# limeorange1102/multimodal-av-model

Hardware: AMD Instinct MI355X
Metric: utterances/sec (4 s clip, 25 fps 96x96 lip) at batch 64, full training step (higher is better)
Workload: dtype bf16; 1 GPU; BASELINE metric configuration (= configs[3]'s per-GPU batch): batch 64/GPU x 4 s (T_audio 64000, T_enc 199, 100 lip frames 96x96 x 2 speakers), wav2vec2-large + ResNet-18 + fusion BiLSTM + CTC + contrastive, fwd+bwd+Adam, random-init weights; variant=as_executed, global_batch=64, parallelism=dp1, audio_passes=2, wav2vec2_regularizers=hf-defaults (dropout 0.1, LayerDrop 0.1, SpecAugment 0.05)

## Files before the change

### include/av_hip.h

```cpp
#ifndef AV_HIP_H
#define AV_HIP_H
#ifdef __cplusplus
extern "C" {
#endif

#define AV_OK 0
#define AV_ERR_ARG 1
#define AV_ERR_LAUNCH 2

#define AV_F32 0
#define AV_BF16 1

#define AV_A_ROWMAJOR 0
#define AV_A_TRANS 1
#define AV_A_CONV2D 2
#define AV_A_CONV3D1 3
#define AV_B_NK 0
#define AV_B_KN 1
#define AV_ACT_NONE 0
#define AV_ACT_GELU 1
#define AV_ACT_MUL_GELU_GRAD 2
#define AV_ACT_GELU_GF 3
#define AV_ACT_MUL_AUX 4

// ... 79 lines not shown
                    int rows_per_batch, int ld, void* stream);
int av_softmax_bwd_rows(const void* p, int pdt, const float* dp, void* ds, int dsdt, long long rows, int cols,
                        float scale, int ld, void* stream);

int av_conv0_ln_gelu(const float* wav, const float* w, const float* bias, const float* gamma, const float* beta, void* out,
                     int out_dtype, int B, int T_in, int L_out, int C, int k, int stride, float eps, void* stream);

int av_lstm_fwd_step(const float* gx, const void* whh, void* hseq, float* cseq, void* gates, void* out_bt, int dtype,
                     int T, int B, int H, int s, void* stream);
int av_lstm_bwd_step(const void* dout, int dout_dtype, long long do_bs, long long do_ts, void* dgates, const void* whhT,
                     const void* gates, const float* cseq, float* dc, int dtype, int T, int B, int H, int s, void* stream);

#define AV_LSTM_COUNTER_INTS 1024
int av_lstm_fwd_layer(const float* gx, const void* whh, void* hseq, float* cseq, void* gates, void* out_bt, int* counters,
                      int T, int B, int H, void* stream);
int av_lstm_bwd_layer(const void* dout, int dout_dtype, long long do_bs, long long do_ts, void* dgates, const void* whhT,
                      const void* gates, const float* cseq, float* dc, int* counters, int T, int B, int H, void* stream);

int av_mask_downsample(const long long* mask, long long* out, int B, int Tin, int Tout, void* stream);
int av_fusion_gather_lerp_fwd(const float* feat, const long long* mask, int* ws_i32, float* out, long long* mask_out,
                              long long* lens, int B, int Ta, int Tv, int D, int groups, void* stream);
int av_fusion_gather_lerp_bwd(const float* dout, const int* ws_i32, float* dfeat, int B, int Ta, int Tv, int D, int groups,
                              void* stream);
int av_permute_bt(const void* in, int idt, void* out, int odt, int B, int T, int D, void* stream);
int av_gather_rows(const void* src, int sdt, const long long* idx, void* out, int odt, long long n, int D, void* stream);
int av_scatter_rows(const float* src, const long long* idx, float* out, long long n, int D, float alpha, int accumulate,
                    void* stream);
int av_class_order(const long long* mask, long long n, long long* order, void* stream);

int av_conv3d_front(const float* x, const void* w, void* y, float* stats, int B, int T, int H, int W, void* stream);
int av_conv3d_front_pool(const float* x, const void* w, void* ymax, void* ymin, float* stats, int B, int T, int H, int W, void* stream);
int av_bn_prelu_minmax(const void* ymax, const void* ymin, const float* scale, const float* shift, const float* slope, void* out, long long n,
                       void* stream);
int av_conv3x3_c64(const void* x, const void* w, void* y, float* stats, int n_img, int H, int W, const float* in_scale,
                   const float* in_shift, const float* in_slope, void* stream);
int av_bn_finalize(const float* partial, int nblk, long long count, const float* gamma, const float* beta,
                   float* running_mean, float* running_var, float momentum, float eps, int training, float* scale,
                   float* shift, int C, double* ws, int ws_zeroed, void* stream);
int av_bn_act(const void* x, const float* scale, const float* shift, const void* res, const float* rscale,
              const float* rshift, const float* slope, void* out, int dtype, long long n, int C, void* stream);
int av_bn_prelu_maxpool(const void* x, const float* scale, const float* shift, const float* slope, void* out, int dtype,
                        long long N, int H, int W, int C, void* stream);
int av_avgpool(const void* x, int dtype, float* out, long long N, int HW, int C, int pm_block, void* stream);

int av_l2norm_fwd(const float* x, float* y, float* nrm, long long rows, int cols, float eps, void* stream);
int av_l2norm_bwd(const float* y, const float* dy, const float* nrm, float* dx, long long rows, int cols, float eps,
                  void* stream);
int av_lse_rows(const float* s, float* lse, float* rowsum, long long rows, int cols, int ld, void* stream);
int av_contrastive_dsim(const float* s, const float* lse, void* out, int odt, long long rows, int cols, int ld, float coef,
                        void* stream);
int av_lse_rows_chunk(const float* s, float* lse, float* rowsum, long long rows, int cols, int ld, int accumulate, void* stream);
int av_contrastive_dsim_chunk(const float* s, const float* lse, void* out, int odt, long long rows, int cols, int ld, float coef,
                              int total_cols, void* stream);
int av_reduce_sum(const float* x, long long n, float* out, float scale, int accumulate, void* stream);
int av_loss_combine(const float* nll, const float* w, const float* c1, const float* c2, float half_lambda, int n, float* out3,
                    void* stream);
int av_ctc_greedy(const float* log_probs, const long long* lengths, int* out_ids, int* out_len, int B, int T, int V, int blank,
                  void* stream);
int av_ctc_beam_workspace_bytes(int B, int T, int V, int beam_width, long long* bytes);
int av_ctc_beam_frame_pass(const float* log_probs, long long stride_b, long long stride_t, const long long* lengths, void* workspace,
                           long long workspace_bytes, int B, int T, int V, int blank, int beam_width, void* stream);
int av_ctc_beam_search(const float* log_probs, long long stride_b, long long stride_t, const long long* lengths, int* out_ids,
                       int* out_len, float* out_score, void* workspace, long long workspace_bytes, int B, int T, int V, int blank,
                       int beam_width, int nbest, void* stream);
int av_ngram_score(const int* ids, const long long* lens, float* out, int B, int Lmax, const float* lm_unigrams, const void* lm_table,
                   long long lm_slots, int lm_order, int lm_vocab, int lm_bos, int lm_probe_bound, void* stream);
// ... 122 lines not shown
```

### multimodal-av-model_amd/_lib.py

```python
from __future__ import annotations

import ctypes as C
import os

from . import precision as _precision

_HERE = os.path.dirname(os.path.abspath(__file__))
LIB_PATH = os.environ.get("AVAMD_LIB") or os.path.join(_HERE, "libavhip.so")

AV_F32, AV_BF16 = 0, 1
A_ROWMAJOR, A_TRANS, A_CONV2D, A_CONV3D1 = 0, 1, 2, 3
B_NK, B_KN = 0, 1
ACT_NONE, ACT_GELU, ACT_MUL_GELU_GRAD, ACT_GELU_GF, ACT_MUL_AUX = 0, 1, 2, 3, 4
LSTM_COUNTER_INTS = 1024

vp, ll, i32, f32 = C.c_void_p, C.c_longlong, C.c_int, C.c_float


class GemmArgs(C.Structure):
    _fields_ = [
        ("A", vp), ("B", vp), ("C", vp), ("C2", vp), ("bias", vp), ("R", vp), ("aux", vp), ("stats", vp),
        ("M", i32), ("N", i32), ("K", i32), ("batch", i32),
        ("lda", ll), ("ldb", ll), ("ldc", ll), ("ldr", ll),
        ("sA", ll), ("sB", ll), ("sC", ll), ("sR", ll), ("sBias", ll),
# ... 52 lines not shown
    "av_log_softmax_bwd_ld": [vp, vp, vp, i32, ll, i32, i32, vp],
    "av_colsum": [vp, i32, vp, ll, i32, ll, i32, vp],
    "av_cast": [vp, i32, vp, i32, ll, vp],
    "av_cast_dropout": [vp, i32, vp, i32, ll, f32, C.c_ulonglong, C.c_uint, vp],
    "av_dropout_uniform": [vp, ll, C.c_ulonglong, C.c_uint, vp],
    "av_fusion_xattn_fwd": [vp, vp, vp, vp, vp, vp, vp, vp, i32, i32, i32, i32, f32, vp],
    "av_fusion_xattn_bwd": [vp, vp, vp, vp, vp, vp, vp, i32, i32, i32, i32, f32, vp],
    "av_zero_feature_cols": [vp, i32, vp, i32, i32, i32, vp],
    "av_overwrite_rows": [vp, i32, vp, vp, ll, i32, vp],
    "av_axpby": [f32, vp, i32, f32, vp, ll, vp],
    "av_mask_rows": [vp, i32, vp, ll, i32, vp],
    "av_mul_scalar_dev": [vp, vp, vp, ll, vp],
    "av_attention_fwd": [vp, vp, vp, vp, vp, i32, i32, i32, i32, i32, i32, ll, ll, ll, ll, ll, ll, ll, ll, vp, f32, f32, C.c_ulonglong, C.c_uint, vp],
    "av_attention_dropmask": [vp, i32, i32, i32, i32, f32, C.c_ulonglong, C.c_uint, vp],
    "av_attention_fwd_mask": [vp, vp, vp, vp, vp, i32, i32, i32, i32, i32, i32, ll, ll, ll, ll, ll, ll, ll, ll, vp, f32, f32, C.c_ulonglong, C.c_uint, vp, vp],
    "av_attention_bwd_mask": [vp, vp, vp, vp, vp, vp, vp, vp, vp, vp, i32, i32, i32, i32, i32, vp, vp, f32, f32, C.c_ulonglong, C.c_uint, vp, vp],
    "av_attention_bwd": [vp, vp, vp, vp, vp, vp, vp, vp, vp, vp, i32, i32, i32, i32, i32, vp, vp, f32, f32, C.c_ulonglong, C.c_uint, vp],
    "av_softmax_rows": [vp, vp, i32, ll, i32, f32, vp, i32, i32, vp],
    "av_conv0_ln_gelu": [vp, vp, vp, vp, vp, vp, i32, i32, i32, i32, i32, i32, i32, f32, vp],
    "av_lstm_fwd_step": [vp, vp, vp, vp, vp, vp, i32, i32, i32, i32, i32, vp],
    "av_lstm_bwd_step": [vp, i32, ll, ll, vp, vp, vp, vp, vp, i32, i32, i32, i32, i32, vp],
    "av_lstm_fwd_layer": [vp, vp, vp, vp, vp, vp, vp, i32, i32, i32, vp],
    "av_lstm_bwd_layer": [vp, i32, ll, ll, vp, vp, vp, vp, vp, vp, i32, i32, i32, vp],
    "av_mask_downsample": [vp, vp, i32, i32, i32, vp],
    "av_fusion_gather_lerp_fwd": [vp, vp, vp, vp, vp, vp, i32, i32, i32, i32, i32, vp],
    "av_fusion_gather_lerp_bwd": [vp, vp, vp, i32, i32, i32, i32, i32, vp],
    "av_permute_bt": [vp, i32, vp, i32, i32, i32, i32, vp],
    "av_gather_rows": [vp, i32, vp, vp, i32, ll, i32, vp],
    "av_scatter_rows": [vp, vp, vp, ll, i32, f32, i32, vp],
    "av_class_order": [vp, ll, vp, vp],
    "av_conv3d_front": [vp, vp, vp, vp, i32, i32, i32, i32, vp],
    "av_conv3d_front_pool": [vp, vp, vp, vp, vp, i32, i32, i32, i32, vp],
    "av_bn_prelu_minmax": [vp, vp, vp, vp, vp, vp, ll, vp],
    "av_conv3x3_c64": [vp, vp, vp, vp, i32, i32, i32, vp, vp, vp, vp],
    "av_bn_finalize": [vp, i32, ll, vp, vp, vp, vp, f32, f32, i32, vp, vp, i32, vp, i32, vp],
    "av_bn_act": [vp, vp, vp, vp, vp, vp, vp, vp, i32, ll, i32, vp],
    "av_bn_prelu_maxpool": [vp, vp, vp, vp, vp, i32, ll, i32, i32, i32, vp],
    "av_avgpool": [vp, i32, vp, ll, i32, i32, i32, vp],
    "av_l2norm_fwd": [vp, vp, vp, ll, i32, f32, vp],
    "av_l2norm_bwd": [vp, vp, vp, vp, ll, i32, f32, vp],
    "av_lse_rows": [vp, vp, vp, ll, i32, i32, vp],
    "av_lse_rows_chunk": [vp, vp, vp, ll, i32, i32, i32, vp],
    "av_contrastive_dsim_chunk": [vp, vp, vp, i32, ll, i32, i32, f32, i32, vp],
    "av_contrastive_dsim": [vp, vp, vp, i32, ll, i32, i32, f32, vp],
    "av_reduce_sum": [vp, ll, vp, f32, i32, vp],
    "av_loss_combine": [vp, vp, vp, vp, f32, i32, vp, vp],
    "av_ctc_greedy": [vp, vp, vp, vp, i32, i32, i32, i32, vp],
    "av_ctc_beam_workspace_bytes": [i32, i32, i32, i32, C.POINTER(ll)],
    "av_ctc_beam_frame_pass": [vp, ll, ll, vp, vp, ll, i32, i32, i32, i32, i32, vp],
    "av_ctc_beam_search": [vp, ll, ll, vp, vp, vp, vp, vp, ll, i32, i32, i32, i32, i32, i32, vp],
    "av_ngram_score": [vp, vp, vp, i32, i32, vp, vp, ll, i32, i32, i32, i32, vp],
    "av_ctc_beam_lm_workspace_bytes": [i32, i32, i32, i32, i32, C.POINTER(ll)],
    "av_ctc_beam_search_lm": [vp, ll, ll, vp, vp, vp, vp, vp, vp, ll, i32, i32, i32, i32, i32, i32, i32, vp, vp, ll, i32, i32, i32, i32, f32, f32, vp],
    "av_context_bias_count": [vp, vp, vp, i32, i32, i32, i32, vp, vp, i32, ll, i32, vp],
    "av_ctc_beam_search_bias": [vp, ll, ll, vp, vp, vp, vp, vp, vp, vp, ll, i32, i32, i32, i32, i32, i32, i32, vp, vp, ll, i32, i32, i32, i32, f32,
                                f32, vp, vp, i32, ll, i32, f32, vp],
    "av_ctc_loss_fwd": [vp, ll, ll, vp, ll, vp, vp, i32, i32, i32, i32, i32, i32, vp, vp, vp, vp],
    "av_ctc_loss_bwd": [vp, ll, ll, vp, ll, vp, vp, i32, i32, i32, i32, i32, vp, vp, vp, vp, vp, vp],
    "av_ctc_nbest_fwd": [vp, ll, ll, vp, ll, ll, vp, vp, i32, i32, i32, i32, i32, i32, vp, vp, vp, vp],
    "av_ctc_nbest_bwd": [vp, ll, ll, vp, ll, ll, vp, vp, i32, i32, i32, i32, i32, i32, vp, vp, vp, vp, vp, vp],
    "av_ctc_align_workspace_bytes": [i32, i32, i32, C.POINTER(ll)],
    "av_ctc_align": [vp, ll, ll, vp, ll, vp, vp, i32, i32, i32, i32, i32, vp, vp, vp, vp, vp, ll, vp],
    "av_error_counts_workspace_bytes": [i32, i32, i32, i32, i32, C.POINTER(ll)],
    "av_error_counts": [vp, ll, vp, vp, ll, ll, vp, i32, i32, i32, i32, i32, i32, vp, vp, i32, i32, vp, vp, ll, vp],
    "av_augment_lips": [vp, vp, vp, i32, i32, i32, i32, C.c_ulonglong, ll, C.c_uint, i32, i32, i32, i32, vp],
    "av_augment_noise": [vp, vp, vp, i32, i32, C.c_ulonglong, ll, f32, f32, vp, vp, vp],
# ... 59 lines not shown
```

### multimodal-av-model_amd/csrc/frontend3d.hip

```cpp
#include "av_common.h"

namespace {

constexpr int KT = 5, KH = 7, KW = 7, TR = KT * KH;
constexpr int KPAD = 288, WLD = 296;
constexpr int TOY = 8, TOX = 16;
constexpr int PH = 2 * TOY + 5, PW = 40;
constexpr int CLD = 68;
constexpr int W_BYTES = 64 * WLD * 2;
constexpr int R2_BYTES = 128 * CLD * 4;
constexpr int R2P_BYTES = 136 * CLD * 4;
constexpr int CARRY_BYTES = 17 * CLD * 4;

struct FrontP {
    const float* x;
    const bf16_t* w;
    bf16_t* y;
    float* stats;
    int T, H, W, Ho, Wo;
    int prefetch;
    bf16_t *ymax, *ymin;
};

template <bool POOL>
__global__ __launch_bounds__(256, 2) void conv3d_front_kernel(const FrontP p) {
    extern __shared__ __attribute__((aligned(16))) char smem[];
    bf16_t* Wl = (bf16_t*)smem;
    bf16_t* patch = (bf16_t*)(smem + W_BYTES);
    float* cs = (float*)(smem + W_BYTES);
    float* carry = (float*)(smem + W_BYTES + R2P_BYTES);
    constexpr int XS = POOL ? 2 : 0;
    const int tid = threadIdx.x, lane = tid & 63, w = tid >> 6;
    const int r = lane & 15, g = lane >> 4;
    int oxt, bt;
    {
        const int nx = gridDim.x, total = nx * gridDim.y;
        const int lin = blockIdx.y * nx + blockIdx.x;
        const int q = total >> 3, rem = total & 7, xcd = lin & 7, slot = lin >> 3;
        const int v = (xcd < rem ? xcd * (q + 1) : rem * (q + 1) + (xcd - rem) * q) + slot;
        bt = v / nx; oxt = v - bt * nx;
    }
    const int t = bt % p.T;
    const int ox0 = oxt * TOX;

    for (int i = tid; i < 64 * KPAD / 8; i += 256) {
        const int row = i / (KPAD / 8), ch = i % (KPAD / 8);
        *(uint4*)(Wl + row * WLD + ch * 8) = *(const uint4*)(p.w + row * KPAD + ch * 8);
    }
    int aoff[9];
#pragma unroll
    for (int ks = 0; ks < 9; ++ks) {
        int tr = 4 * ks + g;
        if (tr > TR - 1) tr = TR - 1;
        const int kt = tr / KH, ky = tr - kt * KH;
        aoff[ks] = (kt * PH + ky) * PW + 2 * r + XS;
    }
    int aoffh[9];
    if constexpr (POOL) {
#pragma unroll
        for (int ks = 0; ks < 9; ++ks) {
            int tr = 4 * ks + g;
            if (tr > TR - 1) tr = TR - 1;
            const int kt = tr / KH, ky = tr - kt * KH;
            aoffh[ks] = (kt * PH + ky + 2 * (r < 8 ? r : 7)) * PW;
        }
    }
    const int ntile = p.Ho / TOY;
    constexpr int NPATCH = KT * PH * (PW / 4), NIT = (NPATCH + 255) / 256;
    float pv[NIT][4];
    auto issue_loads = [&](int oy0) {
#pragma unroll
        for (int it = 0; it < NIT; ++it) {
            const int i = it * 256 + tid;
            const int pc = i % (PW / 4), q = i / (PW / 4);
            const int py = q % PH, kt = q / PH;
            const int ti = t + kt - 2, iy = 2 * oy0 - 3 + py, ix0 = 2 * ox0 - 3 - XS + pc * 4;
            const int tic = ti < 0 ? 0 : (ti > p.T - 1 ? p.T - 1 : ti), iyc = iy < 0 ? 0 : (iy > p.H - 1 ? p.H - 1 : iy);
            const float* src = p.x + ((long long)(bt - t + tic) * p.H + iyc) * p.W;
#pragma unroll
            for (int e = 0; e < 4; ++e) {
                const int ix = ix0 + e;
                const int ixc = ix < 0 ? 0 : (ix > p.W - 1 ? p.W - 1 : ix);
                pv[it][e] = src[ixc];
            }
        }
    };
    auto write_patch = [&](int oy0) {
#pragma unroll
        for (int it = 0; it < NIT; ++it)
            asm volatile("" :: "v"(pv[it][0]), "v"(pv[it][1]), "v"(pv[it][2]), "v"(pv[it][3]));
#pragma unroll
        for (int it = 0; it < NIT; ++it) {
            const int i = it * 256 + tid;
            if (i < NPATCH) {
                const int pc = i % (PW / 4), q = i / (PW / 4);
                const int py = q % PH, kt = q / PH;
                const int ti = t + kt - 2, iy = 2 * oy0 - 3 + py, ix0 = 2 * ox0 - 3 - XS + pc * 4;
                const bool rowok = ti >= 0 && ti < p.T && iy >= 0 && iy < p.H;
                bf16x4 o;
#pragma unroll
                for (int e = 0; e < 4; ++e) o[e] = (bf16_t)((rowok && ix0 + e >= 0 && ix0 + e < p.W) ? pv[it][e] : 0.f);
                *(bf16x4*)(patch + (kt * PH + py) * PW + pc * 4) = o;
            }
        }
    };
    if (p.prefetch) issue_loads(0);
    for (int oyt = 0; oyt < ntile; ++oyt) {
        const int oy0 = oyt * TOY;
        __syncthreads();
        if (!p.prefetch) issue_loads(oy0);
        write_patch(oy0);
        if (p.prefetch && oyt + 1 < ntile) issue_loads(oy0 + TOY);
        __syncthreads();
        f32x4 acc[2][4];
        f32x4 acch = f32x4{0.f, 0.f, 0.f, 0.f};
#pragma unroll
        for (int i = 0; i < 2; ++i)
#pragma unroll
            for (int j = 0; j < 4; ++j) acc[i][j] = f32x4{0.f, 0.f, 0.f, 0.f};
#pragma unroll
        for (int ks = 0; ks < 9; ++ks) {
            bf16x8 b[4];
#pragma unroll
            for (int j = 0; j < 4; ++j) b[j] = *(const bf16x8*)(Wl + (j * 16 + r) * WLD + ks * 32 + 8 * g);
#pragma unroll
            for (int i = 0; i < 2; ++i) {
                const unsigned* ap = (const unsigned*)(patch + aoff[ks] + 2 * (2 * w + i) * PW);
                uint4 av = make_uint4(ap[0], ap[1], ap[2], ap[3]);
                const bf16x8 a = __builtin_bit_cast(bf16x8, av);
#pragma unroll
                for (int j = 0; j < 4; ++j) acc[i][j] = AV_MFMA_F32_16X16X32_LP(a, b[j], acc[i][j], 0, 0, 0);
            }
            if constexpr (POOL) {
                const unsigned* ap = (const unsigned*)(patch + aoffh[ks]);
                uint4 av = make_uint4(ap[0], ap[1], ap[2], ap[3]);
                const bf16x8 bw = *(const bf16x8*)(Wl + (w * 16 + r) * WLD + ks * 32 + 8 * g);
                acch = AV_MFMA_F32_16X16X32_LP(__builtin_bit_cast(bf16x8, av), bw, acch, 0, 0, 0);
            }
        }
        __syncthreads();
#pragma unroll
        for (int i = 0; i < 2; ++i)
#pragma unroll
            for (int j = 0; j < 4; ++j)
#pragma unroll
                for (int e = 0; e < 4; ++e)
                    cs[((2 * w + i) * 16 + 4 * g + e) * CLD + j * 16 + r] = acc[i][j][e];
        if constexpr (POOL) {
            if (g < 2) {
#pragma unroll
                for (int e = 0; e < 4; ++e) cs[(128 + 4 * g + e) * CLD + w * 16 + r] = acch[e];
            }
        }
        __syncthreads();
        if constexpr (POOL) {
            const int pp = tid >> 3, pyl = pp >> 3, pxl = pp & 7, cc = (tid & 7) * 8;
            float mx[8], mn[8];
#pragma unroll
            for (int e = 0; e < 8; ++e) { mx[e] = -INFINITY; mn[e] = INFINITY; }
#pragma unroll
            for (int dy = 0; dy < 3; ++dy) {
                const int ry = 2 * pyl - 1 + dy;
#pragma unroll
                for (int dx = 0; dx < 3; ++dx) {
                    const int cx = 2 * pxl - 1 + dx;
                    const bool ok = (ry >= 0 || oyt > 0) && (cx >= 0 || ox0 > 0);
                    const float* src = ry >= 0 ? (cx >= 0 ? cs + (ry * 16 + cx) * CLD : cs + (128 + ry) * CLD) : carry + (cx + 1) * CLD;
                    const f32x4 v0 = *(const f32x4*)(src + cc), v1 = *(const f32x4*)(src + cc + 4);
#pragma unroll
                    for (int e = 0; e < 4; ++e) {
                        const float a0 = (float)(bf16_t)v0[e], a1 = (float)(bf16_t)v1[e];
                        mx[e] = ok ? fmaxf(mx[e], a0) : mx[e]; mn[e] = ok ? fminf(mn[e], a0) : mn[e];
                        mx[4 + e] = ok ? fmaxf(mx[4 + e], a1) : mx[4 + e]; mn[4 + e] = ok ? fminf(mn[4 + e], a1) : mn[4 + e];
                    }
                }
            }
            bf16x8 omx, omn;
#pragma unroll
            for (int e = 0; e < 8; ++e) { omx[e] = (bf16_t)mx[e]; omn[e] = (bf16_t)mn[e]; }
            const long long po = (((long long)bt * (p.Ho / 2) + oy0 / 2 + pyl) * (p.Wo / 2) + ox0 / 2 + pxl) * 64 + cc;
            *(bf16x8*)(p.ymax + po) = omx;
            *(bf16x8*)(p.ymin + po) = omn;
        } else
        {
            uint4 ov[4];
#pragma unroll
            for (int it = 0; it < 4; ++it) {
                const int id = it * 256 + tid;
                const int pix = id >> 3, cc = (id & 7) * 8;
                const f32x4 v0 = *(const f32x4*)(cs + pix * CLD + cc), v1 = *(const f32x4*)(cs + pix * CLD + cc + 4);
                bf16x8 o;
#pragma unroll
                for (int e = 0; e < 4; ++e) { o[e] = (bf16_t)v0[e]; o[4 + e] = (bf16_t)v1[e]; }
                ov[it] = __builtin_bit_cast(uint4, o);
            }
#pragma unroll
            for (int it = 0; it < 4; ++it) asm volatile("" :: "v"(ov[it].x), "v"(ov[it].y), "v"(ov[it].z), "v"(ov[it].w));
#pragma unroll
            for (int it = 0; it < 4; ++it) {
                const int id = it * 256 + tid;
                const int pix = id >> 3, cc = (id & 7) * 8;
                const int oy = oy0 + (pix >> 4), ox = ox0 + (pix & 15);
                *(uint4*)(p.y + (((long long)bt * p.Ho + oy) * p.Wo + ox) * 64 + cc) = ov[it];
            }
        }
        {
            const int c = tid & 63, rg = tid >> 6;
            float s1 = 0.f, s2 = 0.f;
            if (p.stats)
                for (int rr = rg * 32; rr < rg * 32 + 32; ++rr) { const float v = cs[rr * CLD + c]; s1 += v; s2 += v * v; }
            if (p.stats || POOL) __syncthreads();
            if constexpr (POOL) {
                for (int i = tid; i < 17 * 16; i += 256) {
                    const int px = i >> 4, c4 = (i & 15) * 4;
                    *(f32x4*)(carry + px * CLD + c4) = *(const f32x4*)(cs + (px == 0 ? 135 : 111 + px) * CLD + c4);
// ... 12 lines not shown
        }
    }
}

__global__ __launch_bounds__(256) void bn_prelu_minmax_kernel(const bf16x8* __restrict__ ymax, const bf16x8* __restrict__ ymin, const float* __restrict__ scale,
                                                              const float* __restrict__ shift, const float* __restrict__ slope, bf16x8* __restrict__ out, long long n8) {
    const long long stride = (long long)gridDim.x * blockDim.x;
    long long e = (long long)blockIdx.x * blockDim.x + threadIdx.x;
    const int cg = (int)(e & 7) * 8;
    float sc[8], sh[8], sl[8];
#pragma unroll
    for (int i = 0; i < 8; ++i) { sc[i] = scale[cg + i]; sh[i] = shift[cg + i]; sl[i] = slope[cg + i]; }
    for (; e < n8; e += 4 * stride) {
        bf16x8 a[4], b[4];
#pragma unroll
        for (int u = 0; u < 4; ++u) { const long long i = e + u * stride < n8 ? e + u * stride : e; a[u] = ymax[i]; b[u] = ymin[i]; }
#pragma unroll
        for (int u = 0; u < 4; ++u) {
            if (e + u * stride < n8) {
                bf16x8 o;
#pragma unroll
                for (int i = 0; i < 8; ++i) {
                    float va = (float)a[u][i] * sc[i] + sh[i], vb = (float)b[u][i] * sc[i] + sh[i];
                    va = va >= 0.f ? va : va * sl[i];
                    vb = vb >= 0.f ? vb : vb * sl[i];
                    o[i] = (bf16_t)fmaxf(va, vb);
                }
                out[e + u * stride] = o;
            }
        }
    }
}

}

static int front_launch(const FrontP& p, int B, bool pool, hipStream_t st) {
    static bool done[2] = {false, false};
    const int lds = pool ? W_BYTES + R2P_BYTES + CARRY_BYTES : W_BYTES + R2_BYTES;
    if (!done[pool]) {
        const hipError_t e = pool ? hipFuncSetAttribute((const void*)conv3d_front_kernel<true>, hipFuncAttributeMaxDynamicSharedMemorySize, lds)
                                  : hipFuncSetAttribute((const void*)conv3d_front_kernel<false>, hipFuncAttributeMaxDynamicSharedMemorySize, lds);
        if (e != hipSuccess) {
            av_set_error("av_conv3d_front: cannot raise dynamic LDS to %d", lds);
            return AV_ERR_LAUNCH;
        }
        done[pool] = true;
    }
    dim3 grid((unsigned)(p.Wo / TOX), (unsigned)(B * p.T));
    if (pool) hipLaunchKernelGGL(conv3d_front_kernel<true>, grid, dim3(256), lds, st, p);
    else hipLaunchKernelGGL(conv3d_front_kernel<false>, grid, dim3(256), lds, st, p);
    AV_LAUNCH_CHECK();
    return AV_OK;
}

extern "C" int av_conv3d_front(const float* x, const void* w, void* y, float* stats, int B, int T, int H, int W, void* stream) {
    AV_CHECK(x && w && y && B > 0 && T > 0, "av_conv3d_front: bad args");
    AV_CHECK(H % 16 == 0 && W % 32 == 0, "av_conv3d_front: H=%d must be a multiple of 16 and W=%d of 32", H, W);
    static const int prefetch = [] { const char* e = getenv("AVAMD_FRONT_PREFETCH"); return (e && e[0] == '0') ? 0 : 1; }();
    FrontP p{x, (const bf16_t*)w, (bf16_t*)y, stats, T, H, W, H / 2, W / 2, prefetch, nullptr, nullptr};
    return front_launch(p, B, false, (hipStream_t)stream);
}

extern "C" int av_conv3d_front_pool(const float* x, const void* w, void* ymax, void* ymin, float* stats, int B, int T, int H, int W, void* stream) {
    AV_CHECK(x && w && ymax && ymin && B > 0 && T > 0, "av_conv3d_front_pool: bad args");
    AV_CHECK(H % 16 == 0 && W % 32 == 0, "av_conv3d_front_pool: H=%d must be a multiple of 16 and W=%d of 32", H, W);
    AV_CHECK((uintptr_t)ymax % 16 == 0 && (uintptr_t)ymin % 16 == 0, "av_conv3d_front_pool: outputs must be 16-byte aligned");
    static const int prefetch = [] { const char* e = getenv("AVAMD_FRONT_PREFETCH"); return (e && e[0] == '0') ? 0 : 1; }();
    FrontP p{x, (const bf16_t*)w, nullptr, stats, T, H, W, H / 2, W / 2, prefetch, (bf16_t*)ymax, (bf16_t*)ymin};
    return front_launch(p, B, true, (hipStream_t)stream);
}

extern "C" int av_bn_prelu_minmax(const void* ymax, const void* ymin, const float* scale, const float* shift, const float* slope, void* out,
                                  long long n, void* stream) {
    AV_CHECK(ymax && ymin && scale && shift && slope && out && n >= 0 && n % 64 == 0, "av_bn_prelu_minmax: bad args (n must be a multiple of the 64 channels)");
    AV_CHECK((uintptr_t)ymax % 16 == 0 && (uintptr_t)ymin % 16 == 0 && (uintptr_t)out % 16 == 0, "av_bn_prelu_minmax: 16-byte alignment");
    if (n == 0) return AV_OK;
    const long long n8 = n / 8;
    long long blocks = (n8 + 4 * 256 - 1) / (4 * 256);
    if (blocks > 2048) blocks = 2048;
    hipLaunchKernelGGL(bn_prelu_minmax_kernel, dim3((unsigned)blocks), dim3(256), 0, (hipStream_t)stream, (const bf16x8*)ymax, (const bf16x8*)ymin, scale, shift,
                       slope, (bf16x8*)out, n8);
    AV_LAUNCH_CHECK();
    return AV_OK;
}
```

### multimodal-av-model_amd/model/encoder.py

```python
from __future__ import annotations

import os
from typing import Optional, Union

import torch
import torch.nn as nn

from ..utils import init as _init
from .w2v2 import Wav2Vec2ModelHIP, load_local_config, load_local_weights, w2v2_apply


class AudioEncoder(nn.Module):

    def __init__(self, model_name: Union[str, dict] = "kresnik/wav2vec2-large-xlsr-korean", freeze: bool = True, seed: int = 2,
                 random_init: bool = False):
        super().__init__()
        weights = None
        if isinstance(model_name, dict):
            cfg = model_name
        elif os.path.isdir(model_name):
            cfg = load_local_config(model_name)
            weights = load_local_weights(model_name)
            if weights is None and not random_init:
                raise FileNotFoundError(
# ... 88 lines not shown
        self.output_dim = 512
        self._wcache = {}
        self._nbt = []
        self._bn_ws = None

    def _w(self, conv: nn.Module, dtype):
        p = conv.weight
        key = id(p)
        ver = (p._version, p.data_ptr(), dtype)
        hit = self._wcache.get(key)
        if hit is None or hit[0] != ver:
            with torch.no_grad():
                if p.dim() == 5:
                    w = p.data.reshape(p.shape[0], -1)
                else:
                    w = p.data.permute(0, 2, 3, 1).reshape(p.shape[0], -1)
                hit = (ver, ops.cast(w.contiguous(), dtype))
            self._wcache[key] = hit
        return hit[1]

    def _w_front(self, conv: nn.Module):
        p = conv.weight
        key = ("front", id(p))
        ver = (p._version, p.data_ptr())
        hit = self._wcache.get(key)
        if hit is None or hit[0] != ver:
            with torch.no_grad():
                w = torch.zeros((64, 36, 8), dtype=torch.float32, device=p.device)
                w[:, :35, :7] = p.data.reshape(64, 35, 7)
                hit = (ver, ops.cast(w.reshape(64, 288).contiguous(), compute_dtype()))
            self._wcache[key] = hit
        return hit[1]

    def warm_caches(self, dtype) -> None:
        conv0 = self.frontend3D[0]
        if is_lp(dtype) and tuple(conv0.kernel_size) == (5, 7, 7):
            self._w_front(conv0)
        self._w(conv0, dtype)
        for li in range(1, 5):
            for blk in getattr(self.trunk, f"layer{li}"):
                self._w(blk.conv1, dtype); self._w(blk.conv2, dtype)
                if blk.downsample is not None:
                    self._w(blk.downsample[0], dtype)

    def _bn(self, bn: nn.Module, stats, nblk: int, count: int, training: bool):
        C = bn.num_features
        dev = bn.weight.device
        scale = torch.empty(C, dtype=torch.float32, device=dev); shift = torch.empty(C, dtype=torch.float32, device=dev)
        ws = None
        if training:
            sid = ops.stream()
            if self._bn_ws is None or not isinstance(self._bn_ws, dict):
                self._bn_ws = {}
            ws = self._bn_ws.get(sid)
            if ws is None or ws.device != dev:
                ws = self._bn_ws[sid] = torch.zeros(2 * 1024, dtype=torch.float64, device=dev)
            sync = getattr(self, "_bn_sync", None)
            if sync is not None:
                mode, evs = sync
                i = self._bn_idx
                self._bn_idx += 1
                if mode == "follow" and i < len(evs):
                    torch.cuda.current_stream(dev).wait_event(evs[i])
        L.check(L.lib().av_bn_finalize(ops.ptr(stats), nblk, count, ops.ptr(bn.weight.data), ops.ptr(bn.bias.data),
                                       ops.ptr(bn.running_mean), ops.ptr(bn.running_var), float(bn.momentum), float(bn.eps),
                                       int(training), ops.ptr(scale), ops.ptr(shift), C, ops.ptr(ws), 1, ops.stream()), "av_bn_finalize")
        if training and getattr(self, "_bn_sync", None) is not None and self._bn_sync[0] == "lead":
            ev = torch.cuda.Event(); ev.record()
            self._bn_sync[1].append(ev)
        if training:
# ... 28 lines not shown
                 conv=geo, stats=stats)
        return y, stats, nblk, M, Ho, Wo

    def _act(self, x, scale, shift, slope, res=None, rscale=None, rshift=None):
        out = torch.empty_like(x)
        L.check(L.lib().av_bn_act(ops.ptr(x), ops.ptr(scale), ops.ptr(shift), ops.ptr(res), ops.ptr(rscale), ops.ptr(rshift),
                                  ops.ptr(slope), ops.ptr(out), ops.dt(x), x.numel(), x.shape[-1], ops.stream()), "av_bn_act")
        return out

    @torch.no_grad()
    def _forward_impl(self, x: torch.Tensor) -> torch.Tensor:
        self._nbt = []
        if isinstance(self._bn_ws, dict) and x.is_cuda:
            ws = self._bn_ws.get(ops.stream())
            if ws is not None:
                ws.zero_()
        dtype = compute_dtype()
        training = self.training
        B, C, T, H, W = x.shape
        assert C == 1
        dev = x.device
        conv0 = self.frontend3D[0]
        kt, kh, kw = conv0.kernel_size
        Ho, Wo = (H + 2 * conv0.padding[1] - kh) // conv0.stride[1] + 1, (W + 2 * conv0.padding[2] - kw) // conv0.stride[2] + 1
        M = B * T * Ho * Wo
        fast = (is_lp(dtype) and (kt, kh, kw) == (5, 7, 7) and tuple(conv0.stride) == (1, 2, 2)
                and tuple(conv0.padding) == (2, 3, 3) and H % 16 == 0 and W % 32 == 0)
        N = B * T
        Hp, Wp = (Ho - 1) // 2 + 1, (Wo - 1) // 2 + 1
        pooled = None
        if fast and FRONT_POOL:
            nblk = B * T * (Ho // 8) * (Wo // 16)
            stats = torch.empty((nblk, 2, 64), dtype=torch.float32, device=dev) if training else None
            pooled = torch.empty((2, N * Hp * Wp, 64), dtype=dtype, device=dev)
            L.check(L.lib().av_conv3d_front_pool(ops.ptr(x.contiguous().float()), ops.ptr(self._w_front(conv0)), ops.ptr(pooled[0]), ops.ptr(pooled[1]),
                                                 ops.ptr(stats), B, T, H, W, ops.stream()), "av_conv3d_front_pool")
        elif fast:
            y = torch.empty((M, 64), dtype=dtype, device=dev)
            nblk = B * T * (Ho // 8) * (Wo // 16)
            stats = torch.empty((nblk, 2, 64), dtype=torch.float32, device=dev) if training else None
            L.check(L.lib().av_conv3d_front(ops.ptr(x.contiguous().float()), ops.ptr(self._w_front(conv0)), ops.ptr(y), ops.ptr(stats),
                                            B, T, H, W, ops.stream()), "av_conv3d_front")
        else:
            y = torch.empty((M, 64), dtype=dtype, device=dev)
            xin = ops.cast(x.contiguous().float().view(B, T, H, W), dtype)
            nblk = (M + 127) // 128
            stats = torch.empty((nblk, 2, 64), dtype=torch.float32, device=dev) if training else None
            geo = dict(cT=T, cH=H, cW=W, cCtot=1, cCin=1, cCoff=0, cKt=kt, cKh=kh, cKw=kw, cSh=conv0.stride[1], cSw=conv0.stride[2],
                       cPt=conv0.padding[0], cPh=conv0.padding[1], cPw=conv0.padding[2], cOh=Ho, cOw=Wo)
            ops.gemm(xin, self._w(conv0, dtype), y, M=M, N=64, K=kt * kh * kw, lda=0, ldb=kt * kh * kw, ldc=64, a_mode=L.A_CONV3D1,
                     conv=geo, stats=stats)
        sc, sh = self._bn(self.frontend3D[1], stats, nblk, M, training)
        h = torch.empty((N * Hp * Wp, 64), dtype=dtype, device=dev)
        if pooled is not None:
            L.check(L.lib().av_bn_prelu_minmax(ops.ptr(pooled[0]), ops.ptr(pooled[1]), ops.ptr(sc), ops.ptr(sh), ops.ptr(self.frontend3D[2].weight.data),
                                               ops.ptr(h), h.numel(), ops.stream()), "av_bn_prelu_minmax")
        else:
            L.check(L.lib().av_bn_prelu_maxpool(ops.ptr(y), ops.ptr(sc), ops.ptr(sh), ops.ptr(self.frontend3D[2].weight.data), ops.ptr(h),
                                                ops.dt(h), N, Ho, Wo, 64, ops.stream()), "av_bn_prelu_maxpool")
        Hc, Wc, Cc = Hp, Wp, 64
        FB = 256
        use_pm = POS_MAJOR and is_lp(dtype) and N % FB == 0
        pm_in = 0
        for li in range(1, 5):
            for blk in getattr(self.trunk, f"layer{li}"):
                slope = blk.relu.weight.data
                pm_out = 1 if (use_pm and li >= 2) else 0
                pm1 = pm_in | (pm_out << 1)
                pm2 = pm_out * 3
                if pm_out:
                    c1, st1, nb1, M1, H1, W1 = self._conv2d(h, N, Hc, Wc, Cc, blk.conv1, dtype, training, pm=pm1)
                    s1, b1 = self._bn(blk.bn1, st1, nb1, M1, training)
                    a1 = self._act(c1, s1, b1, slope)
                    c2, st2, nb2, M2, _, _ = self._conv2d(a1, N, H1, W1, blk.conv1.out_channels, blk.conv2, dtype, training, pm=pm2)
                    s2, b2 = self._bn(blk.bn2, st2, nb2, M2, training)
                    if blk.downsample is not None:
                        cd, std, nbd, Md, _, _ = self._conv2d(h, N, Hc, Wc, Cc, blk.downsample[0], dtype, training, pm=pm1)
                        sd, bd = self._bn(blk.downsample[1], std, nbd, Md, training)
                        h = self._act(c2, s2, b2, slope, res=cd, rscale=sd, rshift=bd)
                    else:
                        assert pm_in == pm_out, "position-major trunk: an identity residual needs its input in the layer's pixel order"
                        h = self._act(c2, s2, b2, slope, res=h)
                    Hc, Wc, Cc = H1, W1, blk.conv1.out_channels
                    pm_in = 1
                    continue
                c1, st1, nb1, M1, H1, W1 = self._conv2d(h, N, Hc, Wc, Cc, blk.conv1, dtype, training)
                s1, b1 = self._bn(blk.bn1, st1, nb1, M1, training)
# ... 47 lines not shown
```

Baseline: 1004 utterances/s.

## Store one pooled extreme in lip frontend by gamma sign; vectorise patch loads

```diff
diff --git a/include/av_hip.h b/include/av_hip.h
--- a/include/av_hip.h
+++ b/include/av_hip.h
@@ -135,6 +135,8 @@
 int av_conv3d_front_pool(const float* x, const void* w, void* ymax, void* ymin, float* stats, int B, int T, int H, int W, void* stream);
 int av_bn_prelu_minmax(const void* ymax, const void* ymin, const float* scale, const float* shift, const float* slope, void* out, long long n,
                        void* stream);
+int av_conv3d_front_pool1(const float* x, const void* w, const float* gamma, void* yext, float* stats, int B, int T, int H, int W, void* stream);
+int av_bn_prelu_ext(const void* yext, const float* scale, const float* shift, const float* slope, void* out, long long n, void* stream);
 int av_conv3x3_c64(const void* x, const void* w, void* y, float* stats, int n_img, int H, int W, const float* in_scale,
                    const float* in_shift, const float* in_slope, void* stream);
 int av_bn_finalize(const float* partial, int nblk, long long count, const float* gamma, const float* beta,
diff --git a/multimodal-av-model_amd/_lib.py b/multimodal-av-model_amd/_lib.py
--- a/multimodal-av-model_amd/_lib.py
+++ b/multimodal-av-model_amd/_lib.py
@@ -108,6 +108,8 @@
     "av_conv3d_front": [vp, vp, vp, vp, i32, i32, i32, i32, vp],
     "av_conv3d_front_pool": [vp, vp, vp, vp, vp, i32, i32, i32, i32, vp],
     "av_bn_prelu_minmax": [vp, vp, vp, vp, vp, vp, ll, vp],
+    "av_conv3d_front_pool1": [vp, vp, vp, vp, vp, i32, i32, i32, i32, vp],
+    "av_bn_prelu_ext": [vp, vp, vp, vp, vp, ll, vp],
     "av_conv3x3_c64": [vp, vp, vp, vp, i32, i32, i32, vp, vp, vp, vp],
     "av_bn_finalize": [vp, i32, ll, vp, vp, vp, vp, f32, f32, i32, vp, vp, i32, vp, i32, vp],
     "av_bn_act": [vp, vp, vp, vp, vp, vp, vp, vp, i32, ll, i32, vp],
diff --git a/multimodal-av-model_amd/csrc/frontend3d.hip b/multimodal-av-model_amd/csrc/frontend3d.hip
--- a/multimodal-av-model_amd/csrc/frontend3d.hip
+++ b/multimodal-av-model_amd/csrc/frontend3d.hip
@@ -20,6 +20,7 @@
     int T, H, W, Ho, Wo;
     int prefetch;
     bf16_t *ymax, *ymin;
+    const float* gamma;
 };
 
 template <bool POOL>
@@ -67,50 +68,62 @@
     }
     const int ntile = p.Ho / TOY;
     constexpr int NPATCH = KT * PH * (PW / 4), NIT = (NPATCH + 255) / 256;
-    float pv[NIT][4];
-    auto issue_loads = [&](int oy0) {
+    typedef float f32x4u __attribute__((ext_vector_type(4), aligned(4)));
+    f32x4 pv[NIT];
+    const char* clip = (const char*)(p.x + (long long)(bt - t) * p.H * p.W);
+    const int clipn = p.T * p.H * p.W;
+    auto group_base = [&](int ti, int iy, int ix0) {
+        const int tic = ti < 0 ? 0 : (ti > p.T - 1 ? p.T - 1 : ti), iyc = iy < 0 ? 0 : (iy > p.H - 1 ? p.H - 1 : iy);
+        return (tic * p.H + iyc) * p.W + ix0;
+    };
+    auto issue_loads = [&](int oy0, int lt) {
 #pragma unroll
         for (int it = 0; it < NIT; ++it) {
-            const int i = it * 256 + tid;
+            const int i = it * 256 + lt;
             const int pc = i % (PW / 4), q = i / (PW / 4);
             const int py = q % PH, kt = q / PH;
-            const int ti = t + kt - 2, iy = 2 * oy0 - 3 + py, ix0 = 2 * ox0 - 3 - XS + pc * 4;
-            const int tic = ti < 0 ? 0 : (ti > p.T - 1 ? p.T - 1 : ti), iyc = iy < 0 ? 0 : (iy > p.H - 1 ? p.H - 1 : iy);
-            const float* src = p.x + ((long long)(bt - t + tic) * p.H + iyc) * p.W;
-#pragma unroll
-            for (int e = 0; e < 4; ++e) {
-                const int ix = ix0 + e;
-                const int ixc = ix < 0 ? 0 : (ix > p.W - 1 ? p.W - 1 : ix);
-                pv[it][e] = src[ixc];
-            }
+            const int fb = group_base(t + kt - 2, 2 * oy0 - 3 + py, 2 * ox0 - 3 - XS + pc * 4);
+            const int fbc = fb < 0 ? 0 : (fb > clipn - 4 ? clipn - 4 : fb);
+            pv[it] = *(const f32x4u*)(clip + (unsigned)(fbc * 4));
         }
     };
-    auto write_patch = [&](int oy0) {
+    auto write_patch = [&](int oy0, int lt) {
 #pragma unroll
         for (int it = 0; it < NIT; ++it)
             asm volatile("" :: "v"(pv[it][0]), "v"(pv[it][1]), "v"(pv[it][2]), "v"(pv[it][3]));
 #pragma unroll
         for (int it = 0; it < NIT; ++it) {
-            const int i = it * 256 + tid;
+            const int i = it * 256 + lt;
             if (i < NPATCH) {
                 const int pc = i % (PW / 4), q = i / (PW / 4);
                 const int py = q % PH, kt = q / PH;
                 const int ti = t + kt - 2, iy = 2 * oy0 - 3 + py, ix0 = 2 * ox0 - 3 - XS + pc * 4;
                 const bool rowok = ti >= 0 && ti < p.T && iy >= 0 && iy < p.H;
+                const int fb = group_base(ti, iy, ix0);
+                const int d = fb - (fb < 0 ? 0 : (fb > clipn - 4 ? clipn - 4 : fb));
+                f32x4 v = pv[it];
+                if (d != 0) {
+                    const f32x4 l = v;
+#pragma unroll
+                    for (int e = 0; e < 4; ++e) {
+                        const int j = e + d;
+                        v[e] = j == 0 ? l[0] : j == 1 ? l[1] : j == 2 ? l[2] : j == 3 ? l[3] : 0.f;
+                    }
+                }
                 bf16x4 o;
 #pragma unroll
-                for (int e = 0; e < 4; ++e) o[e] = (bf16_t)((rowok && ix0 + e >= 0 && ix0 + e < p.W) ? pv[it][e] : 0.f);
+                for (int e = 0; e < 4; ++e) o[e] = (bf16_t)((rowok && ix0 + e >= 0 && ix0 + e < p.W) ? v[e] : 0.f);
                 *(bf16x4*)(patch + (kt * PH + py) * PW + pc * 4) = o;
             }
         }
     };
-    if (p.prefetch) issue_loads(0);
+    if (p.prefetch) issue_loads(0, tid);
     for (int oyt = 0; oyt < ntile; ++oyt) {
         const int oy0 = oyt * TOY;
         __syncthreads();
-        if (!p.prefetch) issue_loads(oy0);
-        write_patch(oy0);
-        if (p.prefetch && oyt + 1 < ntile) issue_loads(oy0 + TOY);
+        if (!p.prefetch) issue_loads(oy0, tid);
+        write_patch(oy0, tid);
+        if (p.prefetch && oyt + 1 < ntile) issue_loads(oy0 + TOY, tid);
         __syncthreads();
         f32x4 acc[2][4];
         f32x4 acch = f32x4{0.f, 0.f, 0.f, 0.f};
@@ -165,13 +178,14 @@
                 for (int dx = 0; dx < 3; ++dx) {
                     const int cx = 2 * pxl - 1 + dx;
                     const bool ok = (ry >= 0 || oyt > 0) && (cx >= 0 || ox0 > 0);
-                    const float* src = ry >= 0 ? (cx >= 0 ? cs + (ry * 16 + cx) * CLD : cs + (128 + ry) * CLD) : carry + (cx + 1) * CLD;
+                    const float* src = !ok ? cs + (2 * pyl * 16 + 2 * pxl) * CLD
+                                           : ry >= 0 ? (cx >= 0 ? cs + (ry * 16 + cx) * CLD : cs + (128 + ry) * CLD) : carry + (cx + 1) * CLD;
                     const f32x4 v0 = *(const f32x4*)(src + cc), v1 = *(const f32x4*)(src + cc + 4);
 #pragma unroll
                     for (int e = 0; e < 4; ++e) {
                         const float a0 = (float)(bf16_t)v0[e], a1 = (float)(bf16_t)v1[e];
-                        mx[e] = ok ? fmaxf(mx[e], a0) : mx[e]; mn[e] = ok ? fminf(mn[e], a0) : mn[e];
-                        mx[4 + e] = ok ? fmaxf(mx[4 + e], a1) : mx[4 + e]; mn[4 + e] = ok ? fminf(mn[4 + e], a1) : mn[4 + e];
+                        mx[e] = fmaxf(mx[e], a0); mn[e] = fminf(mn[e], a0);
+                        mx[4 + e] = fmaxf(mx[4 + e], a1); mn[4 + e] = fminf(mn[4 + e], a1);
                     }
                 }
             }
@@ -179,8 +193,15 @@
 #pragma unroll
             for (int e = 0; e < 8; ++e) { omx[e] = (bf16_t)mx[e]; omn[e] = (bf16_t)mn[e]; }
             const long long po = (((long long)bt * (p.Ho / 2) + oy0 / 2 + pyl) * (p.Wo / 2) + ox0 / 2 + pxl) * 64 + cc;
-            *(bf16x8*)(p.ymax + po) = omx;
-            *(bf16x8*)(p.ymin + po) = omn;
+            if (p.gamma) {
+                const f32x4 g0 = *(const f32x4*)(p.gamma + cc), g1 = *(const f32x4*)(p.gamma + cc + 4);
+#pragma unroll
+                for (int e = 0; e < 4; ++e) { omx[e] = g0[e] >= 0.f ? omx[e] : omn[e]; omx[4 + e] = g1[e] >= 0.f ? omx[4 + e] : omn[4 + e]; }
+                *(bf16x8*)(p.ymax + po) = omx;
+            } else {
+                *(bf16x8*)(p.ymax + po) = omx;
+                *(bf16x8*)(p.ymin + po) = omn;
+            }
         } else
         {
             uint4 ov[4];
@@ -259,6 +280,34 @@
     }
 }
 
+__global__ __launch_bounds__(256) void bn_prelu_ext_kernel(const bf16x8* __restrict__ yext, const float* __restrict__ scale, const float* __restrict__ shift,
+                                                           const float* __restrict__ slope, bf16x8* __restrict__ out, long long n8) {
+    const long long stride = (long long)gridDim.x * blockDim.x;
+    long long e = (long long)blockIdx.x * blockDim.x + threadIdx.x;
+    const int cg = (int)(e & 7) * 8;
+    float sc[8], sh[8], sl[8];
+#pragma unroll
+    for (int i = 0; i < 8; ++i) { sc[i] = scale[cg + i]; sh[i] = shift[cg + i]; sl[i] = slope[cg + i]; }
+    for (; e < n8; e += 4 * stride) {
+        bf16x8 a[4];
+#pragma unroll
+        for (int u = 0; u < 4; ++u) a[u] = yext[e + u * stride < n8 ? e + u * stride : e];
+#pragma unroll
+        for (int u = 0; u < 4; ++u) {
+            if (e + u * stride < n8) {
+                bf16x8 o;
+#pragma unroll
+                for (int i = 0; i < 8; ++i) {
+                    float va = (float)a[u][i] * sc[i] + sh[i];
+                    va = va >= 0.f ? va : va * sl[i];
+                    o[i] = (bf16_t)va;
+                }
+                out[e + u * stride] = o;
+            }
+        }
+    }
+}
+
 }
 
 static int front_launch(const FrontP& p, int B, bool pool, hipStream_t st) {
@@ -283,18 +332,42 @@
 extern "C" int av_conv3d_front(const float* x, const void* w, void* y, float* stats, int B, int T, int H, int W, void* stream) {
     AV_CHECK(x && w && y && B > 0 && T > 0, "av_conv3d_front: bad args");
     AV_CHECK(H % 16 == 0 && W % 32 == 0, "av_conv3d_front: H=%d must be a multiple of 16 and W=%d of 32", H, W);
+    AV_CHECK((long long)T * H * W < (1ll << 30), "av_conv3d_front: a clip of T*H*W = %lld pixels is beyond the 2^30 the kernel addresses", (long long)T * H * W);
     static const int prefetch = [] { const char* e = getenv("AVAMD_FRONT_PREFETCH"); return (e && e[0] == '0') ? 0 : 1; }();
-    FrontP p{x, (const bf16_t*)w, (bf16_t*)y, stats, T, H, W, H / 2, W / 2, prefetch, nullptr, nullptr};
+    FrontP p{x, (const bf16_t*)w, (bf16_t*)y, stats, T, H, W, H / 2, W / 2, prefetch, nullptr, nullptr, nullptr};
     return front_launch(p, B, false, (hipStream_t)stream);
 }
 
 extern "C" int av_conv3d_front_pool(const float* x, const void* w, void* ymax, void* ymin, float* stats, int B, int T, int H, int W, void* stream) {
     AV_CHECK(x && w && ymax && ymin && B > 0 && T > 0, "av_conv3d_front_pool: bad args");
     AV_CHECK(H % 16 == 0 && W % 32 == 0, "av_conv3d_front_pool: H=%d must be a multiple of 16 and W=%d of 32", H, W);
+    AV_CHECK((long long)T * H * W < (1ll << 30), "av_conv3d_front_pool: a clip of T*H*W = %lld pixels is beyond the 2^30 the kernel addresses", (long long)T * H * W);
     AV_CHECK((uintptr_t)ymax % 16 == 0 && (uintptr_t)ymin % 16 == 0, "av_conv3d_front_pool: outputs must be 16-byte aligned");
     static const int prefetch = [] { const char* e = getenv("AVAMD_FRONT_PREFETCH"); return (e && e[0] == '0') ? 0 : 1; }();
-    FrontP p{x, (const bf16_t*)w, nullptr, stats, T, H, W, H / 2, W / 2, prefetch, (bf16_t*)ymax, (bf16_t*)ymin};
+    FrontP p{x, (const bf16_t*)w, nullptr, stats, T, H, W, H / 2, W / 2, prefetch, (bf16_t*)ymax, (bf16_t*)ymin, nullptr};
     return front_launch(p, B, true, (hipStream_t)stream);
+}
+
+extern "C" int av_conv3d_front_pool1(const float* x, const void* w, const float* gamma, void* yext, float* stats, int B, int T, int H, int W, void* stream) {
+    AV_CHECK(x && w && gamma && yext && B > 0 && T > 0, "av_conv3d_front_pool1: bad args");
+    AV_CHECK(H % 16 == 0 && W % 32 == 0, "av_conv3d_front_pool1: H=%d must be a multiple of 16 and W=%d of 32", H, W);
+    AV_CHECK((long long)T * H * W < (1ll << 30), "av_conv3d_front_pool1: a clip of T*H*W = %lld pixels is beyond the 2^30 the kernel addresses", (long long)T * H * W);
+    AV_CHECK((uintptr_t)yext % 16 == 0 && (uintptr_t)gamma % 16 == 0, "av_conv3d_front_pool1: gamma and the output must be 16-byte aligned");
+    static const int prefetch = [] { const char* e = getenv("AVAMD_FRONT_PREFETCH"); return (e && e[0] == '0') ? 0 : 1; }();
+    FrontP p{x, (const bf16_t*)w, nullptr, stats, T, H, W, H / 2, W / 2, prefetch, (bf16_t*)yext, nullptr, gamma};
+    return front_launch(p, B, true, (hipStream_t)stream);
+}
+
+extern "C" int av_bn_prelu_ext(const void* yext, const float* scale, const float* shift, const float* slope, void* out, long long n, void* stream) {
+    AV_CHECK(yext && scale && shift && slope && out && n >= 0 && n % 64 == 0, "av_bn_prelu_ext: bad args (n must be a multiple of the 64 channels)");
+    AV_CHECK((uintptr_t)yext % 16 == 0 && (uintptr_t)out % 16 == 0, "av_bn_prelu_ext: 16-byte alignment");
+    if (n == 0) return AV_OK;
+    const long long n8 = n / 8;
+    long long blocks = (n8 + 4 * 256 - 1) / (4 * 256);
+    if (blocks > 2048) blocks = 2048;
+    hipLaunchKernelGGL(bn_prelu_ext_kernel, dim3((unsigned)blocks), dim3(256), 0, (hipStream_t)stream, (const bf16x8*)yext, scale, shift, slope, (bf16x8*)out, n8);
+    AV_LAUNCH_CHECK();
+    return AV_OK;
 }
 
 extern "C" int av_bn_prelu_minmax(const void* ymax, const void* ymin, const float* scale, const float* shift, const float* slope, void* out,
diff --git a/multimodal-av-model_amd/model/encoder.py b/multimodal-av-model_amd/model/encoder.py
--- a/multimodal-av-model_amd/model/encoder.py
+++ b/multimodal-av-model_amd/model/encoder.py
@@ -144,10 +144,21 @@
             self._wcache[key] = hit
         return hit[1]
 
+    def _front_one_extreme(self) -> bool:
+        p = self.frontend3D[2].weight
+        key = ("front1", id(p))
+        ver = (p._version, p.data_ptr())
+        hit = self._wcache.get(key)
+        if hit is None or hit[0] != ver:
+            hit = (ver, bool((p.data >= 0).all().item()))
+            self._wcache[key] = hit
+        return hit[1]
+
     def warm_caches(self, dtype) -> None:
         conv0 = self.frontend3D[0]
         if is_lp(dtype) and tuple(conv0.kernel_size) == (5, 7, 7):
             self._w_front(conv0)
+            self._front_one_extreme()
         self._w(conv0, dtype)
         for li in range(1, 5):
             for blk in getattr(self.trunk, f"layer{li}"):
@@ -242,9 +253,14 @@
         if fast and FRONT_POOL:
             nblk = B * T * (Ho // 8) * (Wo // 16)
             stats = torch.empty((nblk, 2, 64), dtype=torch.float32, device=dev) if training else None
-            pooled = torch.empty((2, N * Hp * Wp, 64), dtype=dtype, device=dev)
-            L.check(L.lib().av_conv3d_front_pool(ops.ptr(x.contiguous().float()), ops.ptr(self._w_front(conv0)), ops.ptr(pooled[0]), ops.ptr(pooled[1]),
-                                                 ops.ptr(stats), B, T, H, W, ops.stream()), "av_conv3d_front_pool")
+            one = self._front_one_extreme()
+            pooled = torch.empty((1 if one else 2, N * Hp * Wp, 64), dtype=dtype, device=dev)
+            if one:
+                L.check(L.lib().av_conv3d_front_pool1(ops.ptr(x.contiguous().float()), ops.ptr(self._w_front(conv0)), ops.ptr(self.frontend3D[1].weight.data),
+                                                      ops.ptr(pooled[0]), ops.ptr(stats), B, T, H, W, ops.stream()), "av_conv3d_front_pool1")
+            else:
+                L.check(L.lib().av_conv3d_front_pool(ops.ptr(x.contiguous().float()), ops.ptr(self._w_front(conv0)), ops.ptr(pooled[0]), ops.ptr(pooled[1]),
+                                                     ops.ptr(stats), B, T, H, W, ops.stream()), "av_conv3d_front_pool")
         elif fast:
             y = torch.empty((M, 64), dtype=dtype, device=dev)
             nblk = B * T * (Ho // 8) * (Wo // 16)
@@ -262,7 +278,10 @@
                      conv=geo, stats=stats)
         sc, sh = self._bn(self.frontend3D[1], stats, nblk, M, training)
         h = torch.empty((N * Hp * Wp, 64), dtype=dtype, device=dev)
-        if pooled is not None:
+        if pooled is not None and pooled.shape[0] == 1:
+            L.check(L.lib().av_bn_prelu_ext(ops.ptr(pooled[0]), ops.ptr(sc), ops.ptr(sh), ops.ptr(self.frontend3D[2].weight.data), ops.ptr(h), h.numel(),
+                                            ops.stream()), "av_bn_prelu_ext")
+        elif pooled is not None:
             L.check(L.lib().av_bn_prelu_minmax(ops.ptr(pooled[0]), ops.ptr(pooled[1]), ops.ptr(sc), ops.ptr(sh), ops.ptr(self.frontend3D[2].weight.data),
                                                ops.ptr(h), h.numel(), ops.stream()), "av_bn_prelu_minmax")
         else:
```

After: 998.5 utterances/s. Within noise of the previous version (-0.6%).
